# zwicker-group/py-pde

Hardware: AMD Instinct MI355X
Metric: Mcells/s (and % HBM roofline) for 3D DiffusionPDE 512^3 fp64; 1/2/4/8-GPU scaling (higher is better)
Workload: dtype f64

## Files before the change

py-pde_amd/csrc/pdehip_euler4_plan.h:

```cpp
#pragma once

#include <cstdio>
#include <cstdlib>

namespace pdehip {
namespace e4plan {

constexpr int TY = 32, TZ = 64, PY = 2, LEVELS = 4, HALO = 4;
constexpr int RY = TY + 2 * HALO, RZ = TZ + 2 * HALO;
constexpr int NPY = RY / PY, NPZ = RZ / 2, PATCHES = NPY * NPZ;
constexpr int THREADS = (PATCHES + 63) / 64 * 64;
constexpr int LROWS = RY + 2, LPITCH = RZ + 4;
constexpr long LDS_BYTES = (long)LEVELS * LROWS * LPITCH * 8;
constexpr int ARR = PATCHES, NARR = LEVELS * PY * 2, GUARD = NPZ;
constexpr int IMAGE = GUARD + NARR * ARR + GUARD;
static_assert(PY == 2 && IMAGE <= LEVELS * LROWS * LPITCH, "the image of the four-step sweep fits its LDS allocation");

constexpr int patch_of_thread(int t) { return t < PATCHES ? t : t - 64; }
static_assert(PATCHES >= 64 && (PATCHES - 64) / NPZ * PY >= HALO + TY, "repeated patches are halo patches");

constexpr int WAVES = THREADS / 64, OWNER_WAVES = 8;
constexpr int wave_levels(int w) { return w < OWNER_WAVES ? LEVELS : w < WAVES - 1 ? LEVELS - 1 : 1; }
constexpr int lane_patch(int t)
{
    const int w = t >> 6, lane = t & 63;
    if (w < OWNER_WAVES) return (HALO / PY + 2 * w + (lane >> 5)) * NPZ + HALO / 2 + (lane & 31);
    if (w == 8) return (HALO / PY + (lane >> 2)) * NPZ + ((lane & 2) ? NPZ - 4 : 0) + (lane & 3);
    if (w == 9) return lane < 40 ? 32 + lane : 648 + (lane - 40);
    if (w == 10) return lane < 40 ? 648 + lane : lane < 48 ? 64 + (lane - 40) : lane;
    return lane < 32 ? lane : PATCHES - 64 + lane;
}
static_assert(TY == 32 && TZ == 64 && PY == 2 && HALO == 4 && WAVES == 12, "lane_patch is written for this tile");
static_assert(OWNER_WAVES * 64 == (TY / PY) * (TZ / 2), "the output patches fill the owner waves exactly");

constexpr int image_index(int level, int row, int cell, int patch) { return GUARD + ((level * PY + row) * 2 + cell) * ARR + patch; }

enum ReadKind { RD_ABOVE0, RD_ABOVE1, RD_BELOW0, RD_BELOW1, RD_LEFT0, RD_LEFT1, RD_RIGHT0, RD_RIGHT1, READ_KINDS };
constexpr int read_index(int level, int kind, int patch)
{
    return kind < RD_BELOW0  ? image_index(level, PY - 1, kind - RD_ABOVE0, patch - NPZ)
         : kind < RD_LEFT0   ? image_index(level, 0, kind - RD_BELOW0, patch + NPZ)
         : kind < RD_RIGHT0  ? image_index(level, kind - RD_LEFT0, 1, patch - 1)
                             : image_index(level, kind - RD_RIGHT0, 0, patch + 1);
}
#define PDEHIP_E4_MINUS_TWICE(x, c) __builtin_fma(-2.0, (c), (x))

constexpr long MIN_CHUNK = 8;
constexpr long WANT_CHUNK = 16;
constexpr long CUS = 256;
static_assert(RY % PY == 0 && HALO % PY == 0 && TZ % 2 == 0 && THREADS <= 1024 && LDS_BYTES <= 160 * 1024, "tile of the four-step sweep");

inline int knob_from_env()
{
    const char *e = getenv("PDEHIP_EULER4");
    if (!e || !e[0]) return -1;
    return e[0] == '0' ? 0 : 1;
}

struct Query {
    int elem;
    int ndim;
    long n0, n1, n2;
    int per[3];
    bool diffusion;
    bool const_faces;
    bool unit;
    int knob;
};

struct Choice {
    bool accepted = false;
    bool unit = false;
    long nty = 0, ntz = 0, nxc = 0, nblocks = 0;
    int lx = 0;
    unsigned block = THREADS;
};

constexpr double DEFAULT_MIN_BYTES = 768.0 * 1048576.0;

inline Choice plan(const Query &q)
{
    Choice c;
    if (q.knob == 0 || !q.diffusion || !q.const_faces) return c;
    if (q.elem != 8 || q.ndim != 3 || q.per[0] != 1 || q.per[1] != 1 || q.per[2] != 1) return c;
    if (q.n1 < TY || q.n1 % TY || q.n2 < TZ || q.n2 % TZ || q.n0 < 2 * HALO + MIN_CHUNK) return c;
    if (q.knob < 0 && (double)q.n0 * (double)q.n1 * (double)q.n2 * 8.0 <= DEFAULT_MIN_BYTES) return c;
    c.nty = q.n1 / TY; c.ntz = q.n2 / TZ;
    const long tiles = c.nty * c.ntz;
    long nxc = (CUS + tiles - 1) / tiles;
    if (nxc > q.n0 / WANT_CHUNK) nxc = q.n0 / WANT_CHUNK;
    if (nxc < 1) nxc = 1;
    const long lx = (q.n0 + nxc - 1) / nxc;
    c.lx = (int)lx;
    c.nxc = (q.n0 + lx - 1) / lx;
    c.nblocks = c.nxc * tiles;
    c.unit = q.unit;
    c.accepted = true;
    return c;
}

inline void format_name(const Choice &c, char *buf, size_t size)
{
    snprintf(buf, size, "euler4_kernel<double,%s> (%dx%d tile, 4 levels in LDS, all-periodic)", c.unit ? "E2_DIFFUSION_UNIT" : "E2_DIFFUSION", TY, TZ);
}

}
}
```

py-pde_amd/csrc/pdehip_kernels_e4.hip:

```cpp
#include <type_traits>

#include "pdehip_common.h"
#include "pdehip_euler2_plan.h"
#include "pdehip_euler4_plan.h"

#ifdef PDEHIP_FAST_VARIANT
#define PDEHIP_VARIANT_NS fastv
#else
#define PDEHIP_VARIANT_NS exactv
#endif
namespace pdehip {
namespace PDEHIP_VARIANT_NS {

#include "pdehip_march4.inc"

int launch_euler4(const NGrid &n, const void *in, void *out, double s1, double s2, const InputBCs &fg, bool const_faces, hipStream_t st, bool *done)
{
    *done = false;
    const int knob = e4plan::knob_from_env();
    if (knob == 0 || e2plan::knobs().off || force_generic_kernels() || n.ndim != 3 || n.dtype != PDEHIP_F64 || in == out) return 0;
    if ((uintptr_t)in % 16 || (uintptr_t)out % 16 || n.off % 2 || n.p[0] % 2 || n.p[1] % 2 || n.p[0] >= (1L << 31)) return 0;
    e4plan::Query q;
    q.elem = 8; q.ndim = n.ndim; q.n0 = n.n[0]; q.n1 = n.n[1]; q.n2 = n.n[2];
    for (int k = 0; k < 3; k++) q.per[k] = classify_axis(fg, k, n.n[k]);
    q.diffusion = true; q.const_faces = const_faces; q.knob = knob;
    q.unit = n.lap_scale[0] == 1.0 && n.lap_scale[1] == 1.0 && n.lap_scale[2] == 1.0 && s1 == 1.0;
    const e4plan::Choice c = e4plan::plan(q);
    if (!c.accepted) return 0;
    LapArgs a;
    memset(&a, 0, sizeof(a));
    a.in = in; a.out = out; a.y = in;
    a.n0 = n.n[0]; a.n1 = n.n[1]; a.n2 = n.n[2];
    a.p0 = n.p[0]; a.p1 = n.p[1]; a.off = n.off;
    a.o_off = n.off; a.o_s0 = a.p0; a.o_s1 = a.p1;
    a.sx = n.lap_scale[0]; a.sy = n.lap_scale[1]; a.sz = n.lap_scale[2];
    a.s1 = s1; a.s2 = s2;
    a.ndim = 3;
    for (int k = 0; k < 3; k++) a.per[k] = 1;
    a.lx = c.lx; a.xstride = c.lx; a.nxc = c.nxc; a.nty = c.nty; a.ntz = c.ntz; a.nblocks = c.nblocks;
    const void *kernel = c.unit ? reinterpret_cast<const void *>(&euler4_kernel<double, E2_DIFFUSION_UNIT>)
                                : reinterpret_cast<const void *>(&euler4_kernel<double, E2_DIFFUSION>);
    char name[160];
    e4plan::format_name(c, name, sizeof(name));
    note_kernel("%s", name);
    void *args[] = {&a};
    PDEHIP_HIP(hipLaunchKernel(kernel, dim3((unsigned)c.nblocks), dim3(c.block), args, 0, st));
    *done = true;
    return 0;
}

int preload_e4_kernels()
{
    hipFuncAttributes attr;
    PDEHIP_HIP(hipFuncGetAttributes(&attr, reinterpret_cast<const void *>(&euler4_kernel<double, E2_DIFFUSION_UNIT>)));
    return 0;
}

}
}
```

py-pde_amd/csrc/pdehip_march4.inc:

```
template <typename T, int M2>
__global__ void __launch_bounds__(e4plan::THREADS) euler4_kernel(const LapArgs a)
{
    static_assert(sizeof(T) == 8 && (M2 == E2_DIFFUSION || M2 == E2_DIFFUSION_UNIT), "fp64 diffusion only");
    using namespace e4plan;
    typedef typename VecT<T, 2>::type V;
    __shared__ __attribute__((aligned(16))) T lds[LEVELS * LROWS * LPITCH];

    const int tid = lane_patch((int)threadIdx.x);
    const int wave = __builtin_amdgcn_readfirstlane((int)threadIdx.x >> 6);
    const int nlev = wave_levels(wave);
    const bool owner = wave < OWNER_WAVES;
    const int py = tid / NPZ, pz = tid - py * NPZ;
    const int ly = py * PY, lz = 2 * pz;

    const long w = xcd_swizzle((long)blockIdx.x, a.nblocks);
    const long tiles = a.nty * a.ntz;
    const long xc = w / tiles, tile = w - xc * tiles;
    const long ty = tile / a.ntz, tz = tile - ty * a.ntz;
    const long x0 = xc * a.xstride;
    const int lx = (int)((a.n0 - x0 < (long)a.lx) ? a.n0 - x0 : (long)a.lx);
    auto wrap = [](long i, long n) { return i < 0 ? i + n : (i >= n ? i - n : i); };

    long roff[PY];
    const long zc = wrap(tz * TZ - HALO + lz, a.n2);
#pragma unroll
    for (int r = 0; r < PY; r++) roff[r] = a.off + wrap(ty * TY - HALO + ly + r, a.n1) * a.p1 + zc;
    const T *in = (const T *)a.in;
    T *out = (T *)a.out;
    auto plane_src = [&](int q) { return wrap(x0 - HALO + q, a.n0) * a.p0; };
    const int qlast = lx + 2 * HALO - 1;
    auto load_plane = [&](int q, V (&dst)[PY]) {
        const long po = plane_src(q < qlast ? q : qlast);
#pragma unroll
        for (int r = 0; r < PY; r++) dst[r] = PDEHIP_LDV((const V *)(in + po + roff[r]));
    };

    const int me = tid;
    int me2 = tid;
    asm volatile("" : "+v"(me2));
    if ((int)threadIdx.x < GUARD) lds[threadIdx.x] = lds[IMAGE - GUARD + threadIdx.x] = 0;

    auto update = [&](double xm, double xp, double up, double dn, double left, double right, double cen) {
        const double dx = PDEHIP_E4_MINUS_TWICE(xm, cen) + xp, dy = PDEHIP_E4_MINUS_TWICE(up, cen) + dn, dz = PDEHIP_E4_MINUS_TWICE(left, cen) + right;
        if (M2 == E2_DIFFUSION_UNIT) return cen + a.s2 * (dx + dy + dz);
        const double ex = dx * a.sx;
        const double ey = dy * a.sy;
        const double ez = dz * a.sz;
        return epilogue<LAP_EULER>(ex + ey + ez, cen, cen, a.s1, a.s2, a.gamma);
    };
    auto fetch = [&](int l, T (&nb)[READ_KINDS]) {
#pragma unroll
        for (int k = 0; k < READ_KINDS; k++) {
            const bool second = k == RD_BELOW1 || k == RD_LEFT1 || k == RD_RIGHT0 || k == RD_RIGHT1;
            nb[k] = lds[read_index(l, k, second ? me2 : me)];
        }
    };
    auto level = [&](const V (&old)[PY], const V (&mid)[PY], const V (&nw)[PY], const T (&nb)[READ_KINDS], V (&res)[PY]) {
        const V above = V{nb[RD_ABOVE0], nb[RD_ABOVE1]}, below = V{nb[RD_BELOW0], nb[RD_BELOW1]};
#pragma unroll
        for (int r = 0; r < PY; r++) {
            const double left = nb[RD_LEFT0 + r], right = nb[RD_RIGHT0 + r];
            const V up = r == 0 ? above : mid[r > 0 ? r - 1 : 0], dn = r == PY - 1 ? below : mid[r < PY - 1 ? r + 1 : r];
            res[r][0] = update(old[r][0], nw[r][0], up[0], dn[0], left, mid[r][1], mid[r][0]);
            res[r][1] = update(old[r][1], nw[r][1], up[1], dn[1], mid[r][0], right, mid[r][1]);
        }
    };
    auto store_level = [&](int l, const V (&pl)[PY]) {
#pragma unroll
        for (int r = 0; r < PY; r++) {
            lds[image_index(l, r, 0, me)] = pl[r][0];
            lds[image_index(l, r, 1, me)] = pl[r][1];
        }
    };

    V R[LEVELS][3][PY], pre[PY];
#pragma unroll
    for (int l = 0; l < LEVELS; l++)
#pragma unroll
        for (int s = 0; s < 3; s++)
#pragma unroll
            for (int r = 0; r < PY; r++) R[l][s][r] = V{0, 0};
    load_plane(0, R[0][0]);
    load_plane(1, R[0][1]);
    load_plane(2, R[0][2]);
#pragma unroll
    for (int l = 0; l < LEVELS; l++) store_level(l, R[l][(4 - l) % 3]);
    __syncthreads();

    auto phase = [&](int i, auto kc) {
        constexpr int K = decltype(kc)::value;
        load_plane(i + 3, pre);
#pragma unroll
        for (int l = 0; l < LEVELS; l++) {
            const V (&old)[PY] = R[l][(K + 3 - l) % 3];
            const V (&mid)[PY] = R[l][(K + 4 - l) % 3];
            const V (&nw)[PY] = R[l][(K + 5 - l) % 3];
            if (l == 0 || l < nlev) {
                T nb[READ_KINDS];
                fetch(l, nb);
                if (l < LEVELS - 1) {
                    level(old, mid, nw, nb, R[l + 1][(K + 4 - l) % 3]);
                } else {
                    V res[PY];
                    level(old, mid, nw, nb, res);
                    const int q = i - 2;
                    if (owner && q >= HALO) {
                        const long po = (x0 + q - HALO) * a.p0;
#pragma unroll
                        for (int r = 0; r < PY; r++) __builtin_nontemporal_store(res[r], (V *)(out + po + roff[r]));
                    }
                }
            }
            __syncthreads();
            if (l <= 1 || l <= nlev) store_level(l, nw);
        }
#pragma unroll
        for (int r = 0; r < PY; r++) R[0][K][r] = pre[r];
    };
    const int iend = lx + 2 * HALO - 3;
    for (int i = 0;; i += 3) {
        phase(i, std::integral_constant<int, 0>());
        if (i + 1 > iend) break;
        phase(i + 1, std::integral_constant<int, 1>());
        if (i + 2 > iend) break;
        phase(i + 2, std::integral_constant<int, 2>());
        if (i + 3 > iend) break;
    }
}
```

Baseline: 1.125 million.

## Double-buffer middle LDS levels to cut per-phase barriers from four to two

Adds a dynamic-LDS ping-pong buffer for levels 1 and 2 of the four-step temporal sweep. Each level's result is written straight into the alternate image and read back in the next phase, so the per-level barrier between compute and store can go. Each phase now has one barrier after level 0 and one at the end instead of one per level. The cost is extra LDS per block, which may lower occupancy, a zero-initialisation pass, and added address arithmetic through pointer swaps.

Result: faster. 1.162 million, median of 6 (+3.3%).

```diff
diff --git a/py-pde_amd/csrc/pdehip_euler4_plan.h b/py-pde_amd/csrc/pdehip_euler4_plan.h
--- a/py-pde_amd/csrc/pdehip_euler4_plan.h
+++ b/py-pde_amd/csrc/pdehip_euler4_plan.h
@@ -43,6 +43,36 @@
          : kind < RD_RIGHT0  ? image_index(level, kind - RD_LEFT0, 1, patch - 1)
                              : image_index(level, kind - RD_RIGHT0, 0, patch + 1);
 }
+
+constexpr int ALT_LEVELS = 2, ALT_LEVEL = GUARD + PY * 2 * ARR + GUARD;
+constexpr int ALT_IMAGE = ALT_LEVELS * ALT_LEVEL;
+constexpr long ALT_BYTES = (long)ALT_IMAGE * 8;
+constexpr int alt_index(int level, int row, int cell, int patch) { return (level - 1) * ALT_LEVEL + GUARD + (row * 2 + cell) * ARR + patch; }
+constexpr int alt_read_index(int level, int kind, int patch)
+{
+    return kind < RD_BELOW0  ? alt_index(level, PY - 1, kind - RD_ABOVE0, patch - NPZ)
+         : kind < RD_LEFT0   ? alt_index(level, 0, kind - RD_BELOW0, patch + NPZ)
+         : kind < RD_RIGHT0  ? alt_index(level, kind - RD_LEFT0, 1, patch - 1)
+                             : alt_index(level, kind - RD_RIGHT0, 0, patch + 1);
+}
+static_assert(LDS_BYTES % 16 == 0 && ALT_BYTES % 16 == 0 && LDS_BYTES + ALT_BYTES <= 160 * 1024, "static and dynamic LDS of the four-step sweep");
+
+enum SchedOp { SCH_STORE, SCH_READ, SCH_BARRIER };
+struct SchedEvent { int op, image, other, interval; };
+constexpr SchedEvent SCHEDULE[] = {
+    {SCH_STORE, 3, 0, 0},
+    {SCH_READ, 0, 0, 0},
+    {SCH_STORE, 1, 1, 0},
+    {SCH_BARRIER, -1, 0, 0},
+    {SCH_STORE, 0, 0, 1},
+    {SCH_READ, 1, 0, 1},
+    {SCH_STORE, 2, 1, 1},
+    {SCH_READ, 2, 0, 1},
+    {SCH_READ, 3, 0, 1},
+    {SCH_BARRIER, -1, 0, 1},
+};
+constexpr int SCHEDULE_EVENTS = sizeof(SCHEDULE) / sizeof(SCHEDULE[0]);
+
 #define PDEHIP_E4_MINUS_TWICE(x, c) __builtin_fma(-2.0, (c), (x))
 
 constexpr long MIN_CHUNK = 8;
diff --git a/py-pde_amd/csrc/pdehip_kernels_e4.hip b/py-pde_amd/csrc/pdehip_kernels_e4.hip
--- a/py-pde_amd/csrc/pdehip_kernels_e4.hip
+++ b/py-pde_amd/csrc/pdehip_kernels_e4.hip
@@ -44,15 +44,20 @@
     e4plan::format_name(c, name, sizeof(name));
     note_kernel("%s", name);
     void *args[] = {&a};
-    PDEHIP_HIP(hipLaunchKernel(kernel, dim3((unsigned)c.nblocks), dim3(c.block), args, 0, st));
+    PDEHIP_HIP(hipLaunchKernel(kernel, dim3((unsigned)c.nblocks), dim3(c.block), args, (size_t)e4plan::ALT_BYTES, st));
     *done = true;
     return 0;
 }
 
 int preload_e4_kernels()
 {
-    hipFuncAttributes attr;
-    PDEHIP_HIP(hipFuncGetAttributes(&attr, reinterpret_cast<const void *>(&euler4_kernel<double, E2_DIFFUSION_UNIT>)));
+    const void *const kernels[] = {reinterpret_cast<const void *>(&euler4_kernel<double, E2_DIFFUSION_UNIT>),
+                                   reinterpret_cast<const void *>(&euler4_kernel<double, E2_DIFFUSION>)};
+    for (const void *kernel : kernels) {
+        PDEHIP_HIP(hipFuncSetAttribute(kernel, hipFuncAttributeMaxDynamicSharedMemorySize, (int)e4plan::ALT_BYTES));
+        hipFuncAttributes attr;
+        PDEHIP_HIP(hipFuncGetAttributes(&attr, kernel));
+    }
     return 0;
 }
 
diff --git a/py-pde_amd/csrc/pdehip_march4.inc b/py-pde_amd/csrc/pdehip_march4.inc
--- a/py-pde_amd/csrc/pdehip_march4.inc
+++ b/py-pde_amd/csrc/pdehip_march4.inc
@@ -5,6 +5,8 @@
     using namespace e4plan;
     typedef typename VecT<T, 2>::type V;
     __shared__ __attribute__((aligned(16))) T lds[LEVELS * LROWS * LPITCH];
+    extern __shared__ __attribute__((aligned(16))) unsigned char euler4_alt[];
+    typedef __attribute__((address_space(3))) T LT;
 
     const int tid = lane_patch((int)threadIdx.x);
     const int wave = __builtin_amdgcn_readfirstlane((int)threadIdx.x >> 6);
@@ -39,6 +41,10 @@
     int me2 = tid;
     asm volatile("" : "+v"(me2));
     if ((int)threadIdx.x < GUARD) lds[threadIdx.x] = lds[IMAGE - GUARD + threadIdx.x] = 0;
+    LT *const alt = (LT *)euler4_alt;
+    LT *cur[ALT_LEVELS] = {(LT *)lds + (image_index(1, 0, 0, 0) - alt_index(1, 0, 0, 0)), (LT *)lds + (image_index(2, 0, 0, 0) - alt_index(2, 0, 0, 0))};
+    LT *oth[ALT_LEVELS] = {alt, alt};
+    for (int k = (int)threadIdx.x; k < ALT_IMAGE; k += THREADS) alt[k] = 0;
 
     auto update = [&](double xm, double xp, double up, double dn, double left, double right, double cen) {
         const double dx = PDEHIP_E4_MINUS_TWICE(xm, cen) + xp, dy = PDEHIP_E4_MINUS_TWICE(up, cen) + dn, dz = PDEHIP_E4_MINUS_TWICE(left, cen) + right;
@@ -73,6 +79,23 @@
         }
     };
 
+    auto fetch_alt = [&](int l, LT *base, T (&nb)[READ_KINDS]) {
+        LT *const b = base + me, *const b2 = base + me2;
+#pragma unroll
+        for (int k = 0; k < READ_KINDS; k++) {
+            const bool second = k == RD_BELOW1 || k == RD_LEFT1 || k == RD_RIGHT0 || k == RD_RIGHT1;
+            nb[k] = (second ? b2 : b)[alt_read_index(l, k, 0)];
+        }
+    };
+    auto store_alt = [&](int l, LT *base, const V (&pl)[PY]) {
+        LT *const b = base + me;
+#pragma unroll
+        for (int r = 0; r < PY; r++) {
+            b[alt_index(l, r, 0, 0)] = pl[r][0];
+            b[alt_index(l, r, 1, 0)] = pl[r][1];
+        }
+    };
+
     V R[LEVELS][3][PY], pre[PY];
 #pragma unroll
     for (int l = 0; l < LEVELS; l++)
@@ -90,6 +113,7 @@
     auto phase = [&](int i, auto kc) {
         constexpr int K = decltype(kc)::value;
         load_plane(i + 3, pre);
+        if (LEVELS - 1 <= nlev) store_level(LEVELS - 1, R[LEVELS - 1][(K + 1) % 3]);
 #pragma unroll
         for (int l = 0; l < LEVELS; l++) {
             const V (&old)[PY] = R[l][(K + 3 - l) % 3];
@@ -97,9 +121,12 @@
             const V (&nw)[PY] = R[l][(K + 5 - l) % 3];
             if (l == 0 || l < nlev) {
                 T nb[READ_KINDS];
-                fetch(l, nb);
+                if (l == 0 || l == LEVELS - 1) fetch(l, nb);
+                else fetch_alt(l, cur[l - 1], nb);
                 if (l < LEVELS - 1) {
-                    level(old, mid, nw, nb, R[l + 1][(K + 4 - l) % 3]);
+                    V (&res)[PY] = R[l + 1][(K + 4 - l) % 3];
+                    level(old, mid, nw, nb, res);
+                    if (l + 1 < LEVELS - 1) store_alt(l + 1, oth[l], res);
                 } else {
                     V res[PY];
                     level(old, mid, nw, nb, res);
@@ -111,11 +138,20 @@
                     }
                 }
             }
-            __syncthreads();
-            if (l <= 1 || l <= nlev) store_level(l, nw);
+            if (l == 0) {
+                __syncthreads();
+                store_level(0, nw);
+            }
         }
+        __syncthreads();
 #pragma unroll
         for (int r = 0; r < PY; r++) R[0][K][r] = pre[r];
+#pragma unroll
+        for (int b = 0; b < ALT_LEVELS; b++) {
+            LT *const t = cur[b];
+            cur[b] = oth[b];
+            oth[b] = t;
+        }
     };
     const int iend = lx + 2 * HALO - 3;
     for (int i = 0;; i += 3) {
```
